# yang-song/score_sde_pytorch

Measured on AMD Instinct MI355X. Metric: pc_sampler_images_per_sec, higher is better.
Workload: dtype f32 via 3-way bf16 split, fp32 accumulate (the 1x1 / NIN / Linear GEMMs and the attention forward as exact-fp32 products on the BF16 matrix pipe, fp32 softmax; 3x3 convolutions and the attention backward on the fp32-MFMA kernels); 1 GPU; configs/ve/cifar10_ncsnpp_continuous PC sampler (reverse_diffusion+langevin), batch 256/GPU, N=1000, 32x32; 1 step = 1 PC iteration = 2 U-Net evaluations; batch_per_gpu=256, sde_steps=1000, state_finite=True, matrix_mode=bf16x6, parallelism=replicas x1 (no collectives)

## Files before the change

### include/ssde.h

```cpp
#ifndef SSDE_H_
#define SSDE_H_

#include <stddef.h>
#include <stdint.h>

#ifdef __cplusplus
extern "C" {
#endif

#define SSDE_ABI_VERSION 13

enum {
  SSDE_PRO_NONE = 0,
  SSDE_PRO_GN = 1,
  SSDE_PRO_GN_SILU = 2,
  SSDE_PRO_SILU = 3
};

typedef struct ssde_src {
  const float* p0;
  const float* p1;
  int32_t c0, c1;
  int32_t pro_mode;
  int32_t gn_groups;
// ... 38 lines not shown
  int64_t wino_ws_floats;
} ssde_conv_args;

enum { SSDE_CONVF_V_GIVEN = 1u,
       SSDE_CONVF_BF16X6 = 2u,
       SSDE_CONVF_NO_KSPLIT = 4u,
       SSDE_CONVF_BKC8 = 8u,
       SSDE_CONVF_GEMM_PIPE = 16u,
       SSDE_CONVF_NO_GEMM_PIPE = 32u,
       SSDE_CONVF_X6_BM64 = 64u,
       SSDE_CONVF_X6_PF2 = 128u,
       SSDE_CONVF_NO_SMALL_COUT = 256u,
       SSDE_CONVF_X6_WIDE = 512u,
       SSDE_CONVF_X6_NO_WIDE = 1024u,
       SSDE_CONVF_KSPLIT2 = 2048u,
       SSDE_CONVF_KSPLIT4 = 4096u };
enum { SSDE_TILE_AUTO = 0, SSDE_TILE_256x64 = 1, SSDE_TILE_128x64 = 2, SSDE_TILE_64x64 = 3, SSDE_TILE_256x32 = 4,
       SSDE_TILE_WINOGRAD = 5,
       SSDE_TILE_WINOGRAD4 = 6,
       SSDE_TILE_WINOGRAD4R = 9,
       SSDE_TILE_WINOGRAD4P = 10 };

typedef struct ssde_gn_stats_args {
  const float* p0; const float* p1; int32_t c0, c1;
  int32_t n, hw, groups; float eps;
  float* mean; float* rstd;
  float* scratch;
  int32_t slices;
  uint32_t flags;
} ssde_gn_stats_args;
enum { SSDE_GNSTATF_ANY_WIDTH = 1u };
// ... 227 lines not shown
} ssde_dsm_loss_args;

typedef struct ssde_sumsq_flat_args { const float* x; int64_t numel; float* partial; float* out; } ssde_sumsq_flat_args;
typedef struct ssde_adam_args {
  float* p; const float* g; float* m; float* v; float* ema;
  int64_t numel;
  const float* hyper;
  const float* gnorm_sq;
} ssde_adam_args;

typedef struct ssde_memset_args { void* dst; int64_t bytes; int32_t value; int32_t _pad0; } ssde_memset_args;

enum { SSDE_PACK_CONV3 = 1, SSDE_PACK_WINO3 = 2, SSDE_PACK_MATRIX = 3, SSDE_PACK_VECTOR = 4,
       SSDE_PACK_WINO4 = 5 ,
       SSDE_PACK_WINO4R = 6 ,
       SSDE_PACK_WINO4P = 7  };
typedef struct ssde_pack_desc {
  const float* src;
  const float* src2;
  float* dst;
  int32_t kind;
  int32_t cout, cin;
  int32_t cout_l, cin_l;
  int32_t flags;
  int32_t r_off, c_off;
  int64_t n;
} ssde_pack_desc;
typedef struct ssde_pack_args { const ssde_pack_desc* table; int32_t count; int32_t kind; int64_t max_n; } ssde_pack_args;
typedef struct ssde_axpy_args {
  const float* x; const float* gate; float* dst; int64_t numel; float alpha; int32_t acc;
} ssde_axpy_args;
// ... 188 lines not shown
```

### score_sde_pytorch_amd/_lib.py

```python
import ctypes as C
import os

_HERE = os.path.dirname(os.path.abspath(__file__))
LIB_PATH = os.environ.get("SSDE_LIB_PATH") or os.path.join(_HERE, "libssde_hip.so")
ABI_VERSION = 13

PRO_NONE, PRO_GN, PRO_GN_SILU, PRO_SILU = 0, 1, 2, 3
TILE_AUTO, TILE_256x64, TILE_128x64, TILE_64x64, TILE_256x32, TILE_WINOGRAD, TILE_WINOGRAD4 = 0, 1, 2, 3, 4, 5, 6
TILE_WINOGRAD4R = 9
TILE_WINOGRAD4P = 10
TILES_WINOGRAD4 = (TILE_WINOGRAD4, TILE_WINOGRAD4R, TILE_WINOGRAD4P)
CONVF_V_GIVEN, CONVF_BF16X6, CONVF_NO_KSPLIT, CONVF_BKC8, CONVF_GEMM_PIPE, CONVF_NO_GEMM_PIPE, CONVF_X6_BM64, CONVF_X6_PF2, \
    CONVF_NO_SMALL_COUT, CONVF_X6_WIDE, CONVF_X6_NO_WIDE, CONVF_KSPLIT2, CONVF_KSPLIT4 = 1, 2, 4, 8, 16, 32, 64, 128, 256, 512, 1024, 2048, 4096
WGRADF_DIRECT, WGRADF_F2, WGRADF_F4_FORCE, WGRADF_NO_STREAMK, WGRADF_NO_XCD_ORDER, WGRADF_1X1_CHUNKED, WGRADF_XVEC1 = 1, 2, 4, 8, 16, 32, 64
GNBWDF_THREE_KERNELS, GNBWDF_DEFER_PARAMS = 1, 2
(OP_CONV, OP_GN_STATS, OP_UPFIRDN, OP_ATTN, OP_EMBED, OP_TO_NHWC, OP_TO_NCHW, OP_BIAS_ACT, OP_SUMSQ,
 OP_RANDN, OP_LANGEVIN, OP_PREDICTOR, OP_FILL, OP_STEP_INC, OP_WGRAD, OP_COLSUM, OP_GN_BWD_REDUCE, OP_PROLOGUE_BWD,
 OP_ATTN_BWD, OP_PERTURB, OP_DSM_LOSS, OP_SUMSQ_FLAT, OP_ADAM, OP_MEMSET, OP_AXPY, OP_PACK, OP_PROJECT,
 OP_GN_FINALIZE, OP_PF_DRIFT, OP_HUTCH_DIV, OP_COLSUM_FINISH, OP_GN_BWD_FINISH, OP_GN_APPLY, OP_GN_APPLY_BWD) = range(1, 35)
GNSTATF_ANY_WIDTH = 1
FIRF_GENERAL, FIRF_TILED = 1, 2
FIR_MAX_TAPS = 16
FINISH_JOBS = 16
COLSUMF_DEFER = 1
PACK_CONV3, PACK_WINO3, PACK_MATRIX, PACK_VECTOR, PACK_WINO4, PACK_WINO4R, PACK_WINO4P = 1, 2, 3, 4, 5, 6, 7

_fp = C.c_void_p


class Src(C.Structure):
    _fields_ = [("p0", _fp), ("p1", _fp), ("c0", C.c_int32), ("c1", C.c_int32),
                ("pro_mode", C.c_int32), ("gn_groups", C.c_int32),
                ("gn_mean", _fp), ("gn_rstd", _fp), ("gn_gamma", _fp), ("gn_beta", _fp),
                ("drop_thresh", C.c_uint32), ("drop_scale", C.c_float), ("drop_seed", _fp),
                ("drop_salt", C.c_uint32), ("_pad", C.c_int32)]


class ConvArgs(C.Structure):
    _fields_ = [("main", Src), ("aux", Src), ("w_main", _fp), ("w_aux", _fp),
                ("n", C.c_int32), ("h_in", C.c_int32), ("w_in", C.c_int32),
# ... 439 lines not shown
```

### score_sde_pytorch_amd/csrc/backward.hip

```cpp
#include "ssde_common.h"

namespace {

inline unsigned grid_for(size_t total, int block = 256, unsigned cap = 256 * 16) {
  size_t b = (total + block - 1) / block;
  if (b < 1) b = 1;
  return (unsigned)(b > cap ? cap : b);
}

__global__ __launch_bounds__(256) void colsum_kernel(const float* __restrict__ g, int g_ld, int g_off, int hw, int c,
                                                     float scale, float* __restrict__ out, int out_ld, int out_off) {
  SSDE_LDS(smem);
  float4* red = reinterpret_cast<float4*>(smem);
  const int n = blockIdx.z, slices = gridDim.y, slice = blockIdx.y;
  const int cl = blockIdx.x * 64 + (threadIdx.x & 63);
  const int pl = threadIdx.x >> 6;
  const int col = g_off + cl * 4;
  const int per_slice = (hw + slices - 1) / slices;
  const int p0 = slice * per_slice, p1 = min(hw, p0 + per_slice);
  float4 s = make_float4(0.f, 0.f, 0.f, 0.f);
  if (cl * 4 < c && col + 4 <= g_ld) {
    const float* base = g + (size_t)n * hw * g_ld + col;
    int px = p0 + pl;
    for (; px + 12 < p1; px += 16) {
// ... 871 lines not shown
        const float u = (float)(t[a][0] * G[b][0] + t[a][1] * G[b][1] + t[a][2] * G[b][2]);
        if (kForm == 0) {
          d.dst[(((r * 8 + wv) * 9 + j) * 32 + (cs & 31)) * 4 + e] = u;
        } else if (kForm == 2) {
          d.dst[(((size_t)pos * nq + c4) * ((size_t)ntl * 64) + co) * 4 + e] = u;
        } else {
          const int lane = (e >> 1) * 32 + (cs & 31), half = cs >> 5;
          const int w = pos < 32 ? (pos >> 2) : 2 * (pos - 32) + half;
          const size_t base = (r * 8 + w) * (size_t)(9 * 32 * 4);
          d.dst[base + (pos < 32 ? ((pos & 3) * 64 + lane) * 4 + half * 2 + (e & 1) : 1024 + lane * 2 + (e & 1))] = u;
        }
      }
  }
}

__global__ __launch_bounds__(256) void pack_matrix_kernel(const ssde_pack_desc* __restrict__ table) {
  const ssde_pack_desc d = table[blockIdx.y];
  const int ld = (d.cout_l + 63) / 64 * 64;
  for (size_t idx = (size_t)blockIdx.x * 256 + threadIdx.x; idx < (size_t)d.n; idx += (size_t)gridDim.x * 256) {
    const int i = (int)(idx / d.cin), j = (int)(idx % d.cin);
    const int row = ((d.flags & 1) ? j : i) + d.r_off, col = ((d.flags & 1) ? i : j) + d.c_off;
    d.dst[((size_t)(col >> 3) * ld + row) * 8 + (col & 7)] = d.src[idx];
  }
}

__global__ __launch_bounds__(256) void pack_vector_kernel(const ssde_pack_desc* __restrict__ table) {
  const ssde_pack_desc d = table[blockIdx.y];
  for (size_t idx = (size_t)blockIdx.x * 256 + threadIdx.x; idx < (size_t)d.n; idx += (size_t)gridDim.x * 256)
    d.dst[d.r_off + idx] = d.src[idx] + (d.src2 ? d.src2[idx] : 0.f);
}

}

extern "C" int ssde_pack_weights(const ssde_pack_args* a, void* stream) {
  SSDE_REQUIRE(a && a->table && a->count > 0 && a->max_n > 0, "pack_weights: bad args");
  size_t bx = ((size_t)a->max_n + 255) / 256;
  if (bx > 256) bx = 256;
  const dim3 grid((unsigned)bx, (unsigned)a->count);
  hipStream_t st = static_cast<hipStream_t>(stream);
  switch (a->kind) {
    case SSDE_PACK_CONV3: hipLaunchKernelGGL(pack_conv3_kernel, grid, dim3(256), 0, st, a->table); break;
    case SSDE_PACK_WINO3: hipLaunchKernelGGL(pack_wino3_kernel, grid, dim3(256), 0, st, a->table); break;
    case SSDE_PACK_WINO4: hipLaunchKernelGGL(pack_wino4_kernel<0>, grid, dim3(256), 0, st, a->table); break;
    case SSDE_PACK_WINO4R: hipLaunchKernelGGL(pack_wino4_kernel<1>, grid, dim3(256), 0, st, a->table); break;
    case SSDE_PACK_WINO4P: hipLaunchKernelGGL(pack_wino4_kernel<2>, grid, dim3(256), 0, st, a->table); break;
    case SSDE_PACK_MATRIX: hipLaunchKernelGGL(pack_matrix_kernel, grid, dim3(256), 0, st, a->table); break;
    case SSDE_PACK_VECTOR: hipLaunchKernelGGL(pack_vector_kernel, grid, dim3(256), 0, st, a->table); break;
    default: ssde_set_error("pack_weights: unknown kind %d", a->kind); return SSDE_EINVAL;
  }
  SSDE_LAUNCH_CHECK();
  return SSDE_OK;
}
```

### score_sde_pytorch_amd/csrc/conv1x1.hip

```cpp
#include "ssde_common.h"

typedef float f32x16 __attribute__((ext_vector_type(16)));

#ifdef SSDE_GEMM_TRACE
__device__ unsigned long long* g_gemm_trace;
extern "C" int ssde_debug_gemm_trace(void* buf) {
  return hipMemcpyToSymbol(HIP_SYMBOL(g_gemm_trace), &buf, sizeof(buf)) == hipSuccess ? 0 : -5;
}
#define SSDE_GT(slot)                                                                  \
  do {                                                                                 \
    if (gt_on) g_gemm_trace[(slot)] = __builtin_amdgcn_s_memtime();                    \
  } while (0)
__device__ unsigned long long* g_gemm_wg_trace;
extern "C" int ssde_debug_gemm_wg_trace(void* buf) {
  return hipMemcpyToSymbol(HIP_SYMBOL(g_gemm_wg_trace), &buf, sizeof(buf)) == hipSuccess ? 0 : -5;
}
#define SSDE_GW(slot)                                                                                          \
  do {                                                                                                         \
    if (threadIdx.x == 0 && g_gemm_wg_trace != nullptr) {                                                      \
      g_gemm_wg_trace[(size_t)blockIdx.x * 4 + (slot)] = __builtin_amdgcn_s_memtime();                         \
      if ((slot) == 0) g_gemm_wg_trace[(size_t)blockIdx.x * 4 + 3] = __builtin_amdgcn_s_getreg((4 << 0) | (0 << 6) | (31 << 11)) | ((unsigned long long)__builtin_amdgcn_s_getreg((20 << 0) | (0 << 6) | (3 << 11)) << 32); \
    }                                                                                                          \
  } while (0)
#else
// ... 197 lines not shown
    SSDE_GT(41 + half * 2);
    __syncthreads();
    SSDE_GT(42 + half * 2);
  }
}

#ifndef SSDE_X6_PF2_OCC_LOSS
#define SSDE_X6_PF2_OCC_LOSS 1
#endif
constexpr int XBK = 16;
template <int kBM, int kBN = 128> struct X6 {
  static constexpr int kPlaneA = kBM * XBK * 2, kPlaneB = kBN * XBK * 2;
  static constexpr int kStageBytes = 3 * kPlaneA + 3 * kPlaneB;
  static constexpr int NA = kBM / 64;
  static constexpr int NBW = kBN / 64;
};

template <bool kGn, int kBM, int kPF, int kBN = 128>
__global__ __launch_bounds__(kThreads, kBN == 256 ? 2 : (kBM == 64 ? 4 : 3) - (kPF == 2 ? SSDE_X6_PF2_OCC_LOSS : 0)) void gemm1x1_bf16x6_kernel(const GemmParams p) {
  using X = X6<kBM, kBN>;
  constexpr int NA = X::NA, NB = X::NBW, NBW = X::NBW, RS = 64;
  SSDE_LDS(smem);
  char* lds = reinterpret_cast<char*>(smem);
  const int tid = threadIdx.x, wave = tid >> 6, lane = tid & 63;
  const int li = lane & 31, lh = lane >> 5;
  const int xcd = blockIdx.x & 7, lin = blockIdx.x >> 3;
  const int nt = lin % p.n_tiles, mt = (lin / p.n_tiles) * 8 + xcd;
#ifdef SSDE_GEMM_TRACE
  const bool gt_on = tid == 0 && blockIdx.x == 0 && g_gemm_trace != nullptr;
#endif
  SSDE_GT(0);
  if (mt >= p.m_tiles) return;
  SSDE_GW(0);
  const int m0 = mt * kBM, n0 = nt * kBN;
  const int wm0 = (wave >> 1) * (kBM / 2), wn0 = (wave & 1) * (kBN / 2);
  const ssde_src& s = p.src;
  SsdePro pro = ssde_pro_decode(s);
  pro.gn = kGn;
  const int Ctot = s.c0 + s.c1;
  const int cpg = kGn ? Ctot / s.gn_groups : 1;
  const int nst = (p.K + XBK - 1) / XBK;
  const int ncin8 = (p.K + 7) >> 3;

  const int f = tid & 3, r0 = tid >> 2;
  int arow[NA], aimg[NA];
  bool aok[NA];
#pragma unroll
  for (int i = 0; i < NA; ++i) {
    const int m = m0 + r0 + i * RS;
    aok[i] = m < p.M;
    arow[i] = aok[i] ? m : 0;
    aimg[i] = arow[i] / p.HW;
  }
  bool bok[NB];
#pragma unroll
  for (int i = 0; i < NB; ++i) bok[i] = (n0 + r0 + i * RS) < p.CoutPad;
  const float* bptr = p.wpk + ((size_t)n0 + r0) * 8 + (f & 1) * 4;

  struct ARegs { float4 av[NA]; };
  struct StageRegs {
    float4 bv[NB];
    float mu[NA], rs[NA];
    float4 gam, bet;
  };
  auto load_a = [&](int st, ARegs& A) __attribute__((always_inline)) {
    const int c_base = st * XBK;
    const bool second = c_base >= s.c0;
    const float* base = second ? s.p1 : s.p0;
    const int C = second ? s.c1 : s.c0;
    const int cthr = (second ? c_base - s.c0 : c_base) + f * 4;
    const float* ap = base + (c_base + f * 4 < p.K ? cthr : 0);
#pragma unroll
    for (int i = 0; i < NA; ++i) A.av[i] = *reinterpret_cast<const float4*>(ap + (size_t)arow[i] * C);
  };
  auto load_rest = [&](int st, StageRegs& R) __attribute__((always_inline)) {
    const int c_cur = st * XBK + f * 4;
    const int cin8 = min(st * 2 + (f >> 1), ncin8 - 1);
    const float* bp = bptr + (size_t)cin8 * p.CoutPad * 8;
#pragma unroll
    for (int i = 0; i < NB; ++i) R.bv[i] = *reinterpret_cast<const float4*>(bp + (bok[i] ? i * RS * 8 : 0));
    R.gam = make_float4(1.f, 1.f, 1.f, 1.f); R.bet = make_float4(0.f, 0.f, 0.f, 0.f);
#pragma unroll
    for (int i = 0; i < NA; ++i) { R.mu[i] = 0.f; R.rs[i] = 1.f; }
    if (kGn) {
      const int cg = c_cur < p.K ? c_cur : 0;
      R.gam = *reinterpret_cast<const float4*>(s.gn_gamma + cg);
      R.bet = *reinterpret_cast<const float4*>(s.gn_beta + cg);
#pragma unroll
      for (int i = 0; i < NA; ++i) {
        const int gi = aimg[i] * s.gn_groups + cg / cpg;
        R.mu[i] = s.gn_mean[gi];
        R.rs[i] = s.gn_rstd[gi];
      }
    }
  };
  auto store_stage = [&](int st, const ARegs& A, const StageRegs& R, char* buf) __attribute__((always_inline)) {
    const int cin8 = st * 2 + (f >> 1);
    const int c_cur = st * XBK + f * 4;
    const bool k_ok = c_cur < p.K;
    uint2 q0, q1, q2;
#pragma unroll
    for (int i = 0; i < NA; ++i) {
      float4 v = make_float4(0.f, 0.f, 0.f, 0.f);
      if (aok[i] && k_ok)
        v = ssde_pro_apply(A.av[i], R.mu[i], R.rs[i], R.gam, R.bet, (uint32_t)arow[i] * (uint32_t)Ctot + (uint32_t)c_cur, pro);
      char* d = buf + (r0 + i * RS) * (XBK * 2) + f * 8;
      ssde_split3(v, q0, q1, q2);
      *reinterpret_cast<uint2*>(d) = q0;
      *reinterpret_cast<uint2*>(d + X::kPlaneA) = q1;
      *reinterpret_cast<uint2*>(d + 2 * X::kPlaneA) = q2;
    }
#pragma unroll
    for (int i = 0; i < NB; ++i) {
      float4 w = make_float4(0.f, 0.f, 0.f, 0.f);
      if (bok[i] && cin8 < ncin8) w = R.bv[i];
      char* d = buf + 3 * X::kPlaneA + (r0 + i * RS) * (XBK * 2) + f * 8;
      ssde_split3(w, q0, q1, q2);
      *reinterpret_cast<uint2*>(d) = q0;
      *reinterpret_cast<uint2*>(d + X::kPlaneB) = q1;
      *reinterpret_cast<uint2*>(d + 2 * X::kPlaneB) = q2;
    }
  };

  f32x16 acc[NA][NBW];
#pragma unroll
  for (int a = 0; a < NA; ++a)
#pragma unroll
    for (int b = 0; b < NBW; ++b)
#pragma unroll
      for (int r = 0; r < 16; ++r) acc[a][b][r] = 0.f;
  const int aoff = (wm0 + li) * (XBK * 2) + lh * 16, boff = 3 * X::kPlaneA + (wn0 + li) * (XBK * 2) + lh * 16;
  auto mfma_stage = [&](const char* cur) __attribute__((always_inline)) {
    ssde_u32x4 A[NA][3];
#pragma unroll
    for (int q = 0; q < 3; ++q)
#pragma unroll
// ... 226 lines not shown
  auto run_tile = [&](int vb, f32x16 (&acc)[2][2], f32x16 (&old)[2][2]) __attribute__((always_inline)) {
    const int xcd = vb & 7, lin = vb >> 3;
    const int nt = lin % p.n_tiles, mt = (lin / p.n_tiles) * 8 + xcd;
    const int m0 = mt * BM, n0 = nt * BN;
    int arow[NI], aimg[NI];
    bool aok[NI], bok[NI];
#pragma unroll
    for (int i = 0; i < NI; ++i) {
      const int m = m0 + r0 + i * RS;
      aok[i] = m < p.M;
      arow[i] = aok[i] ? m : 0;
      aimg[i] = arow[i] / p.HW;
      bok[i] = (n0 + r0 + i * RS) < p.CoutPad;
    }
    const float* bptr = p.wpk + ((size_t)n0 + r0) * 8 + (f & 1) * 4;
    float4 av[NI], bv[NI];
    float mu[NI] = {0.f, 0.f}, rs[NI] = {1.f, 1.f};
    float4 gam = make_float4(1.f, 1.f, 1.f, 1.f), bet = make_float4(0.f, 0.f, 0.f, 0.f);
    auto load_stage = [&](int st) __attribute__((always_inline)) {
      const int c_base = st * KB;
      const bool second = c_base >= s.c0;
      const float* base = second ? s.p1 : s.p0;
      const int C = second ? s.c1 : s.c0;
      const int cthr = (second ? c_base - s.c0 : c_base) + f * 4;
      const int c_cur = c_base + f * 4;
      const float* ap = base + (c_cur < p.K ? cthr : 0);
#pragma unroll
      for (int i = 0; i < NI; ++i) av[i] = *reinterpret_cast<const float4*>(ap + (size_t)arow[i] * C);
      const int cin8 = min(st * 2 + (f >> 1), ncin8 - 1);
      const float* bp = bptr + (size_t)cin8 * p.CoutPad * 8;
#pragma unroll
      for (int i = 0; i < NI; ++i) bv[i] = *reinterpret_cast<const float4*>(bp + (bok[i] ? i * RS * 8 : 0));
      if (kGn) {
        const int cg = c_cur < p.K ? c_cur : 0;
        gam = *reinterpret_cast<const float4*>(s.gn_gamma + cg);
        bet = *reinterpret_cast<const float4*>(s.gn_beta + cg);
#pragma unroll
        for (int i = 0; i < NI; ++i) {
          const int gi = aimg[i] * s.gn_groups + cg / cpg;
          mu[i] = s.gn_mean[gi];
          rs[i] = s.gn_rstd[gi];
        }
      }
    };
    auto store_stage = [&](int st, char* buf) __attribute__((always_inline)) {
      const int cin8 = st * 2 + (f >> 1), c_cur = st * KB + f * 4;
      const bool k_ok = c_cur < p.K;
#pragma unroll
      for (int i = 0; i < NI; ++i) {
        float4 v = make_float4(0.f, 0.f, 0.f, 0.f);
        if (aok[i] && k_ok)
          v = ssde_pro_apply(av[i], mu[i], rs[i], gam, bet, (uint32_t)arow[i] * (uint32_t)Ctot + (uint32_t)c_cur, pro);
        float4 w = make_float4(0.f, 0.f, 0.f, 0.f);
        if (bok[i] && cin8 < ncin8) w = bv[i];
        if constexpr (kX6) {
          using X = X6<128>;
          uint2 q0, q1, q2;
          char* d = buf + (r0 + i * RS) * (KB * 2) + f * 8;
          ssde_split3(v, q0, q1, q2);
          *reinterpret_cast<uint2*>(d) = q0;
          *reinterpret_cast<uint2*>(d + X::kPlaneA) = q1;
          *reinterpret_cast<uint2*>(d + 2 * X::kPlaneA) = q2;
          ssde_split3(w, q0, q1, q2);
          *reinterpret_cast<uint2*>(d + 3 * X::kPlaneA) = q0;
          *reinterpret_cast<uint2*>(d + 3 * X::kPlaneA + X::kPlaneB) = q1;
          *reinterpret_cast<uint2*>(d + 3 * X::kPlaneA + 2 * X::kPlaneB) = q2;
        } else {
          float* fb = reinterpret_cast<float*>(buf);
          float* d = fb + (r0 + i * RS) * LDK + f * 4;
          *reinterpret_cast<float2*>(d) = make_float2(v.x, v.y);
          *reinterpret_cast<float2*>(d + 2) = make_float2(v.z, v.w);
          float* e = fb + (BM + r0 + i * RS) * LDK + f * 4;
          *reinterpret_cast<float2*>(e) = make_float2(w.x, w.y);
          *reinterpret_cast<float2*>(e + 2) = make_float2(w.z, w.w);
        }
      }
    };
    auto mfma_stage = [&](const char* cur) __attribute__((always_inline)) {
      if constexpr (kX6) {
        using X = X6<128>;
        const int aoff = (wm0 + li) * (KB * 2) + lh * 16, boff = 3 * X::kPlaneA + (wn0 + li) * (KB * 2) + lh * 16;
        ssde_u32x4 A[2][3], B[2][3];
#pragma unroll
        for (int q = 0; q < 3; ++q)
#pragma unroll
          for (int a = 0; a < 2; ++a) {
            A[a][q] = *reinterpret_cast<const ssde_u32x4*>(cur + aoff + q * X::kPlaneA + a * 32 * (KB * 2));
            B[a][q] = *reinterpret_cast<const ssde_u32x4*>(cur + boff + q * X::kPlaneB + a * 32 * (KB * 2));
          }
// ... 92 lines not shown
  g->gn = s.pro_mode == SSDE_PRO_GN || s.pro_mode == SSDE_PRO_GN_SILU;
  SSDE_REQUIRE(a->w_aux && a->dst, "conv1x1: null weights / destination");
  GemmParams& p = g->p;
  p.src = s; p.wpk = a->w_aux;
  p.M = a->n * a->h_out * a->w_out; p.HW = a->h_out * a->w_out; p.K = s.c0 + s.c1;
  p.Cout = a->c_out; p.CoutPad = ssde_cdiv(a->c_out, 64) * 64;
  p.m_tiles = ssde_cdiv(p.M, BM); p.n_tiles = ssde_cdiv(a->c_out, BN);
  ssde_fill_epilogue(p, a);
  const bool gn_ok = a->c_out % 4 == 0 && (p.HW % 64 == 0 || (p.HW >= 8 && p.HW < 64 && 64 % p.HW == 0));
  SSDE_REQUIRE(!a->gn_part || gn_ok, "conv1x1: GroupNorm partials need H*W %% 64 == 0 or a power of two in 8..32");
  pl->gn_slices = !gn_ok ? 0 : p.HW % 64 == 0 ? (p.HW / 64) * 4 : 4;
  pl->ws_floats = 0;
  p.lHW = ssde_ilog2(p.HW);
  p.gn_entries = p.HW >= 64 ? a->n * (p.HW / 64) : a->n;
  const bool x6 = g->x6 = (a->flags & SSDE_CONVF_BF16X6) != 0;
  {
    const int total = ssde_cdiv(p.m_tiles, 8) * 8 * p.n_tiles;
    const int wgs = (2 * ssde_num_cus() + 7) / 8 * 8;
    const bool pipe_ok = !(a->flags & SSDE_CONVF_NO_GEMM_PIPE) && a->c_out % 4 == 0 && (!a->gn_part || p.HW % 64 == 0) && (!a->chan_add || p.HW % 8 == 0);
    const bool wide_first = a->c_out >= 512 && a->c_out % 256 == 0 && !(a->flags & (SSDE_CONVF_X6_NO_WIDE | SSDE_CONVF_X6_BM64 | SSDE_CONVF_X6_PF2)) &&
                            (long long)ssde_cdiv(p.M, 128) * (a->c_out / 256) >= 2ll * ssde_num_cus();
    const bool pays = x6 && p.K >= 512 && (long long)p.m_tiles * p.n_tiles > wgs && !wide_first;
    g->pipe = pipe_ok && x6 && (pays || (a->flags & SSDE_CONVF_GEMM_PIPE));
    if (g->pipe) {
      pl->lds_bytes = 2 * X6<128>::kStageBytes + 4 * kSlabFloats * 4;
      g->grid = total < wgs ? total : wgs;
      return SSDE_OK;
    }
  }
  int xbm = 128, xpf = 1, xbn = BN;
// ... 25 lines not shown
bool ssde_conv1x1_wants(const ssde_conv_args* a) {
  if (a->ksize != 0 || a->aux.p0 == nullptr || a->tile != SSDE_TILE_AUTO) return false;
  const long long M = (long long)a->n * a->h_out * a->w_out;
  return a->c_out >= 96 && M >= 128 && M < (1ll << 31);
}

int ssde_conv1x1_plan(const ssde_conv_args* a, ssde_conv_plan* pl) {
  GemmPlan g;
  return gemm_plan(a, &g, pl);
}

int ssde_conv1x1_launch(const ssde_conv_args* a, hipStream_t st) {
  GemmPlan g;
  ssde_conv_plan pl;
  if (int rc = gemm_plan(a, &g, &pl)) return rc;
  const int lds = pl.lds_bytes;
  const bool gn = g.gn;
  if (g.pipe) return gn ? gemm_go<gemm1x1_pipe_kernel<true, true>>(g, lds, st) : gemm_go<gemm1x1_pipe_kernel<false, true>>(g, lds, st);
  if (!g.x6) return gn ? gemm_go<gemm1x1_kernel<true>>(g, lds, st) : gemm_go<gemm1x1_kernel<false>>(g, lds, st);
  if (g.xbn == 256) return gn ? gemm_go<gemm1x1_bf16x6_kernel<true, 128, 1, 256>>(g, lds, st) : gemm_go<gemm1x1_bf16x6_kernel<false, 128, 1, 256>>(g, lds, st);
  if (g.xbm == 128 && g.xpf == 1) return gn ? gemm_go<gemm1x1_bf16x6_kernel<true, 128, 1>>(g, lds, st) : gemm_go<gemm1x1_bf16x6_kernel<false, 128, 1>>(g, lds, st);
  if (g.xbm == 128) return gn ? gemm_go<gemm1x1_bf16x6_kernel<true, 128, 2>>(g, lds, st) : gemm_go<gemm1x1_bf16x6_kernel<false, 128, 2>>(g, lds, st);
  if (g.xpf == 1) return gn ? gemm_go<gemm1x1_bf16x6_kernel<true, 64, 1>>(g, lds, st) : gemm_go<gemm1x1_bf16x6_kernel<false, 64, 1>>(g, lds, st);
  return gn ? gemm_go<gemm1x1_bf16x6_kernel<true, 64, 2>>(g, lds, st) : gemm_go<gemm1x1_bf16x6_kernel<false, 64, 2>>(g, lds, st);
}
```

### score_sde_pytorch_amd/engine.py

```python
import ctypes as C
import math
import os
from typing import Callable, NamedTuple

import numpy as np
import torch

from . import _lib as L

_FLT = 4
INV_SQRT2 = float(1.0 / np.sqrt(2.0))

FC_OTHER, FC_CONV3, FC_CONV1, FC_ATTN, FC_GN, FC_FIR = 0, 1, 2, 3, 4, 5

W4P_MIN_BATCH = 16


class Buf:
    __slots__ = ("shape", "numel", "name", "persistent", "tensor", "first", "last")

    def __init__(self, shape, name="", persistent=False):
        self.shape = tuple(int(s) for s in shape)
        self.numel = int(np.prod(self.shape))
        self.name = name
# ... 111 lines not shown
                    free.append(b.tensor)
        self.blocks = blocks
        self.arena_bytes = sum(t.numel() for t in blocks) * _FLT
        ops, classes, flops, starts = [], [], [], []
        for si, (kind, fields, fclass, fl) in enumerate(self.specs):
            starts.append(len(ops))
            if si in fused_fir:
                if fused_fir[si] is None:
                    continue
                fields = dict(fields, dst2=fused_fir[si])
            for sub_fields, sub_class, sub_fl in _expand(kind, fields, fclass, fl):
                args = L.ARGS[kind]()
                _fill(args, sub_fields)
                if kind in _ROUTE and "flags" not in sub_fields:
                    args.flags = _ROUTE[kind]()
                ops.append(L.make_op(kind, args, sub_class))
                classes.append(sub_class)
                flops.append(sub_fl)
        prog = Program(L.op_array(ops), classes, flops, self)
        prog.spec_start = starts + [len(ops)]
        return prog


def _fir_pairs(specs):
    out = {}
    if os.environ.get("SSDE_FUSE_FIR", "1") == "0":
        return out
    same = ("n", "h_in", "w_in", "c", "h_out", "w_out", "up", "down", "pad0", "pad1", "kh", "kw", "k")
    for i in range(len(specs) - 1):
        (k0, f0, _, _), (k1, f1, _, _) = specs[i], specs[i + 1]
# ... 178 lines not shown
    c4, nt = (w.shape[1] + 3) // 4, (w.shape[0] + 63) // 64
    v = _wino4_u(w).reshape(nt, 2, 32, c4, 2, 2, 36)
    fp = v[..., :32].reshape(nt, 2, 32, c4, 2, 2, 8, 4).permute(3, 0, 6, 7, 4, 2, 1, 5).reshape(c4, nt, 8, 4 * 64 * 4)
    hp = v[..., 32:].permute(3, 0, 6, 1, 4, 2, 5).reshape(c4, nt, 8, 64 * 2)
    return torch.cat([fp, hp], dim=3).contiguous()


def pack_wino4p_weight(w):
    return _wino4_u(w).unflatten(1, (-1, 4)).permute(3, 1, 0, 2).contiguous()


def pack_matrix(w):
    return pack_conv_weight(w.reshape(w.shape[0], w.shape[1], 1, 1))


class Conv3Route(NamedTuple):
    name: str
    tile: int
    pack_kind: int
    pack: Callable
    takes_v: bool
    needs_ws: bool


DIRECT = Conv3Route("direct", L.TILE_AUTO, L.PACK_CONV3, pack_conv_weight, False, False)
F2 = Conv3Route("f2", L.TILE_WINOGRAD, L.PACK_WINO3, pack_wino_weight, False, False)
F4 = Conv3Route("f4", L.TILE_WINOGRAD4, L.PACK_WINO4, pack_wino4_weight, True, False)
F4R = Conv3Route("f4r", L.TILE_WINOGRAD4R, L.PACK_WINO4R, pack_wino4r_weight, True, False)
F4P = Conv3Route("f4p", L.TILE_WINOGRAD4P, L.PACK_WINO4P, pack_wino4p_weight, False, True)
CONV3_ROUTES = (DIRECT, F2, F4, F4R, F4P)
# ... 65 lines not shown
                w = w.to(torch.float32)
                w = w.t() if tr else w.reshape(w.shape[0], -1)
                ms.append(w)
            m = torch.cat(ms, dim=0) if len(ms) > 1 else ms[0]
            if cin_pad and m.shape[1] < cin_pad:
                m = torch.nn.functional.pad(m, (0, cin_pad - m.shape[1]))
            return m
        rows, desc = 0, []
        for p_, tr in parts:
            n_rows = p_.shape[1] if tr else p_.shape[0]
            cin = p_.shape[0] if tr else int(np.prod(p_.shape[1:]))
            desc.append(dict(param=p_, row0=rows, rows=n_rows, transpose=tr))
            rows += n_rows
        meta = dict(kind="matrix", sources=params, logical=logical, parts=desc, cin_store=cin,
                    dims=(rows, max(cin, cin_pad or 0)))
        recipe = [dict(kind=L.PACK_MATRIX, src=d["param"], cout=d["param"].shape[0], cin=int(np.prod(d["param"].shape[1:])),
                       cout_l=rows, cin_l=0, flags=int(d["transpose"]), r_off=d["row0"], c_off=0, n="src") for d in desc]
        return self.add(params, lambda *ws: pack_matrix(logical(*ws)), meta, recipe)

    def vector(self, params, mode="cat", pad_to=None):
        def fn(*vs):
            vs = [v.to(torch.float32) for v in vs]
            x = torch.cat(vs) if mode == "cat" else sum(vs[1:], vs[0])
            if pad_to and x.numel() < pad_to:
                x = torch.nn.functional.pad(x, (0, pad_to - x.numel()))
            return x.clone()
        off, desc = 0, []
        for p_ in params:
            desc.append(dict(param=p_, off=0 if mode == "sum" else off, n=p_.numel()))
            off += p_.numel()
        if mode == "sum":
            assert len(params) == 2
            recipe = [dict(kind=L.PACK_VECTOR, src=params[0], src2=params[1], r_off=0, n="src")]
        else:
            recipe = [dict(kind=L.PACK_VECTOR, src=d["param"], r_off=d["off"], n="src") for d in desc]
        return self.add(params, fn, dict(kind="vector", mode=mode, sources=list(params), parts=desc), recipe)

    def derived(self, packed, route=None):
        meta = self.meta[id(packed)]
        key = (id(packed), route)
        if key not in self.meta:
            cout_l, cin_l = meta["dims"]
            if meta["kind"] == "conv3":
                p_ = meta["sources"][0]
                fn = lambda w: route.pack(w.permute(1, 0, 2, 3).flip(2, 3))
                recipe = [dict(kind=route.pack_kind, src=p_, cout=p_.shape[0], cin=p_.shape[1],
                               cout_l=cin_l, cin_l=cout_l, flags=1, n="dst")]
            else:
                fn = lambda m: pack_matrix(m.t().contiguous())
                recipe = [dict(kind=L.PACK_MATRIX, src=d["param"], cout=d["param"].shape[0], cin=int(np.prod(d["param"].shape[1:])),
                               cout_l=cin_l, cin_l=0, flags=int(not d["transpose"]), r_off=0, c_off=d["row0"], n="src")
                          for d in meta["parts"]]
            self.meta[key] = self.add(meta["sources"], lambda *ws: fn(meta["logical"](*ws)), None, recipe)
        return self.meta[key]

    def _source_addresses(self):
        return tuple(s.data_ptr() for e in self.entries if e.recipe is not None for s in e.sources)

    def _build_tables(self):
        descs = {}
        for e in self.entries:
            packed, recipe = e.packed, e.recipe
            if recipe is None:
                continue
            for r in recipe:
                d = L.PackDesc()
                src = r["src"]
                d.src, d.dst, d.kind = src.data_ptr(), packed.data_ptr(), r["kind"]
# ... 662 lines not shown
```

### score_sde_pytorch_amd/hipops.py

```python
import ctypes as C

import numpy as np
import torch

from . import _lib as L
from .engine import F4R, conv3_route_of_tile, pack_conv_weight, pack_matrix, wino4_v_floats


def _stream():
    return C.c_void_p(torch.cuda.current_stream().cuda_stream)


def _need_cuda(*ts):
    for t in ts:
        if t is not None and not t.is_cuda:
            raise RuntimeError("score_sde_pytorch_amd HIP op called with a %s tensor (no CPU fallback)" % t.device.type)


def _p(t):
    return None if t is None else t.data_ptr()


def _fill_src(s, t, t2=None, pro=L.PRO_NONE, gn=None):
    s.p0, s.c0 = _p(t), t.shape[-1]
# ... 51 lines not shown
    _fill_drop(a.src, drop)
    sums = torch.empty(n, gn[4], 2, device=x.device)
    scratch = torch.empty(n * slices * c * 2, device=x.device)
    dgamma, dbeta = torch.empty(c, device=x.device), torch.empty(c, device=x.device)
    a.acc0, a.acc1 = int(g0 is not None), int(g1 is not None)
    g0 = torch.empty_like(x) if g0 is None else g0
    g1 = (torch.empty_like(x2) if g1 is None else g1) if x2 is not None else None
    a.dy, a.n, a.hw, a.sums, a.dgamma, a.dbeta, a.scratch, a.slices = _p(dy), n, hw, _p(sums), _p(dgamma), _p(dbeta), _p(scratch), slices
    a.g0, a.g1 = _p(g0), _p(g1)
    L.check(L.load().ssde_gn_apply_bwd(C.byref(a), _stream()), "ssde_gn_apply_bwd")
    return g0, g1, dgamma, dbeta


def conv2d(x=None, weight=None, bias=None, stride=1, pad=1, x2=None, pro=L.PRO_NONE, gn=None,
           aux=None, aux2=None, aux_weight=None, aux_pro=L.PRO_NONE, aux_gn=None,
           chan_add=None, resid=None, scale=1.0, tile=L.TILE_AUTO, out_hw=None, flags=None, pad_end=0):
    _need_cuda(x, aux, resid)
    a = L.ConvArgs()
    keep = []
    route = conv3_route_of_tile(tile)
    if x is not None:
        n, h_in, w_in = x.shape[0], x.shape[1], x.shape[2]
        c_out = weight.shape[0]
        h_out = (h_in + 2 * pad + pad_end - 3) // stride + 1
        w_out = (w_in + 2 * pad + pad_end - 3) // stride + 1
        if out_hw is not None:
            h_out, w_out = out_hw
        _fill_src(a.main, x, x2, pro, gn)
        wp = route.pack(weight.to(x.device)); keep.append(wp)
        if route is F4R:
            wv = torch.empty(wino4_v_floats(n, h_in, w_in, x.shape[-1] + (x2.shape[-1] if x2 is not None else 0)), device=x.device)
            keep.append(wv)
            a.wino_v = _p(wv)
        a.w_main, a.ksize, a.stride, a.pad, a.h_in, a.w_in = _p(wp), 3, stride, pad, h_in, w_in
        a.pad_end = pad_end
    else:
        n, h_out, w_out = aux.shape[0], aux.shape[1], aux.shape[2]
        c_out = aux_weight.shape[0]
        a.ksize, a.stride, a.pad = 0, 1, 0
    if aux is not None:
        _fill_src(a.aux, aux, aux2, aux_pro, aux_gn)
        wa = pack_matrix(aux_weight.to(aux.device)); keep.append(wa)
        a.w_aux = _p(wa)
    dev = (x if x is not None else aux).device
    dst = torch.empty(n, h_out, w_out, c_out, device=dev)
    a.n, a.h_out, a.w_out, a.c_out, a.tile = n, h_out, w_out, c_out, tile
    a.bias = _p(bias)
    if chan_add is not None:
        a.chan_add, a.chan_add_ld = _p(chan_add), chan_add.shape[-1]
    a.resid, a.out_scale, a.dst = _p(resid), scale, _p(dst)
    a.flags = L.conv_route_flags() if flags is None else flags
    if route.needs_ws:
        need = int(L.load().ssde_conv_ws_floats(C.byref(a)))
        L.check(min(need, 0), "ssde_conv_ws_floats")
        ws = torch.empty(need, device=dev); keep.append(ws)
        a.wino_ws, a.wino_ws_floats = _p(ws), need
    L.check(L.load().ssde_conv2d(C.byref(a), _stream()), "ssde_conv2d")
    return dst


def upfirdn2d_nhwc(x, kernel, up=1, down=1, pad=(0, 0), pro=L.PRO_NONE, gn=None, dual=False, accumulate_into=None, flags=0):
    _need_cuda(x)
    n, h, w, c = x.shape
    kh, kw = kernel.shape
    if not (1 <= kh <= L.FIR_MAX_TAPS and 1 <= kw <= L.FIR_MAX_TAPS):
        raise ValueError("upfirdn2d: a %dx%d kernel; at most %d taps per axis" % (kh, kw, L.FIR_MAX_TAPS))
# ... 297 lines not shown
```

Before: 5.589 images/s.

## Pre-split 1x1 GEMM weights into bf16x3 planes at pack time

The weight packer now also writes three bf16 split planes (hi, mid, lo) in a per-stage layout next to the fp32 packed matrix. The bf16x6 1x1 GEMM kernels load those planes with 16-byte vector reads and copy them straight into LDS, so they no longer run the per-stage ssde_split3 on weights inside the hot loop. This cuts ALU work and simplifies the B-operand staging, but adds weight memory, a flag that must be set when packing, and a hard error when it is missing.

```diff
diff --git a/include/ssde.h b/include/ssde.h
--- a/include/ssde.h
+++ b/include/ssde.h
@@ -76,7 +76,8 @@
        SSDE_CONVF_X6_WIDE = 512u,
        SSDE_CONVF_X6_NO_WIDE = 1024u,
        SSDE_CONVF_KSPLIT2 = 2048u,
-       SSDE_CONVF_KSPLIT4 = 4096u };
+       SSDE_CONVF_KSPLIT4 = 4096u,
+       SSDE_CONVF_W_AUX_X6 = 8192u };
 enum { SSDE_TILE_AUTO = 0, SSDE_TILE_256x64 = 1, SSDE_TILE_128x64 = 2, SSDE_TILE_64x64 = 3, SSDE_TILE_256x32 = 4,
        SSDE_TILE_WINOGRAD = 5,
        SSDE_TILE_WINOGRAD4 = 6,
@@ -334,7 +335,8 @@
 enum { SSDE_PACK_CONV3 = 1, SSDE_PACK_WINO3 = 2, SSDE_PACK_MATRIX = 3, SSDE_PACK_VECTOR = 4,
        SSDE_PACK_WINO4 = 5 ,
        SSDE_PACK_WINO4R = 6 ,
-       SSDE_PACK_WINO4P = 7  };
+       SSDE_PACK_WINO4P = 7 ,
+       SSDE_PACK_MATRIX_X6 = 8 };
 typedef struct ssde_pack_desc {
   const float* src;
   const float* src2;
diff --git a/score_sde_pytorch_amd/_lib.py b/score_sde_pytorch_amd/_lib.py
--- a/score_sde_pytorch_amd/_lib.py
+++ b/score_sde_pytorch_amd/_lib.py
@@ -12,6 +12,7 @@
 TILES_WINOGRAD4 = (TILE_WINOGRAD4, TILE_WINOGRAD4R, TILE_WINOGRAD4P)
 CONVF_V_GIVEN, CONVF_BF16X6, CONVF_NO_KSPLIT, CONVF_BKC8, CONVF_GEMM_PIPE, CONVF_NO_GEMM_PIPE, CONVF_X6_BM64, CONVF_X6_PF2, \
     CONVF_NO_SMALL_COUT, CONVF_X6_WIDE, CONVF_X6_NO_WIDE, CONVF_KSPLIT2, CONVF_KSPLIT4 = 1, 2, 4, 8, 16, 32, 64, 128, 256, 512, 1024, 2048, 4096
+CONVF_W_AUX_X6 = 8192
 WGRADF_DIRECT, WGRADF_F2, WGRADF_F4_FORCE, WGRADF_NO_STREAMK, WGRADF_NO_XCD_ORDER, WGRADF_1X1_CHUNKED, WGRADF_XVEC1 = 1, 2, 4, 8, 16, 32, 64
 GNBWDF_THREE_KERNELS, GNBWDF_DEFER_PARAMS = 1, 2
 (OP_CONV, OP_GN_STATS, OP_UPFIRDN, OP_ATTN, OP_EMBED, OP_TO_NHWC, OP_TO_NCHW, OP_BIAS_ACT, OP_SUMSQ,
@@ -23,7 +24,7 @@
 FIR_MAX_TAPS = 16
 FINISH_JOBS = 16
 COLSUMF_DEFER = 1
-PACK_CONV3, PACK_WINO3, PACK_MATRIX, PACK_VECTOR, PACK_WINO4, PACK_WINO4R, PACK_WINO4P = 1, 2, 3, 4, 5, 6, 7
+PACK_CONV3, PACK_WINO3, PACK_MATRIX, PACK_VECTOR, PACK_WINO4, PACK_WINO4R, PACK_WINO4P, PACK_MATRIX_X6 = 1, 2, 3, 4, 5, 6, 7, 8
 
 _fp = C.c_void_p
 
diff --git a/score_sde_pytorch_amd/csrc/backward.hip b/score_sde_pytorch_amd/csrc/backward.hip
--- a/score_sde_pytorch_amd/csrc/backward.hip
+++ b/score_sde_pytorch_amd/csrc/backward.hip
@@ -909,13 +909,24 @@
   }
 }
 
+template <bool kX6>
 __global__ __launch_bounds__(256) void pack_matrix_kernel(const ssde_pack_desc* __restrict__ table) {
   const ssde_pack_desc d = table[blockIdx.y];
   const int ld = (d.cout_l + 63) / 64 * 64;
+  uint16_t* planes = reinterpret_cast<uint16_t*>(d.dst + (size_t)((d.cin_l + 7) >> 3) * ld * 8);
   for (size_t idx = (size_t)blockIdx.x * 256 + threadIdx.x; idx < (size_t)d.n; idx += (size_t)gridDim.x * 256) {
     const int i = (int)(idx / d.cin), j = (int)(idx % d.cin);
     const int row = ((d.flags & 1) ? j : i) + d.r_off, col = ((d.flags & 1) ? i : j) + d.c_off;
-    d.dst[((size_t)(col >> 3) * ld + row) * 8 + (col & 7)] = d.src[idx];
+    const float w = d.src[idx];
+    d.dst[((size_t)(col >> 3) * ld + row) * 8 + (col & 7)] = w;
+    if (kX6) {
+      uint2 q0, q1, q2;
+      ssde_split3(make_float4(w, 0.f, 0.f, 0.f), q0, q1, q2);
+      uint16_t* o = planes + ((size_t)(col >> 4) * 3 * ld + row) * 16 + (col & 15);
+      o[0] = (uint16_t)q0.x;
+      o[(size_t)ld * 16] = (uint16_t)q1.x;
+      o[(size_t)ld * 32] = (uint16_t)q2.x;
+    }
   }
 }
 
@@ -939,7 +950,8 @@
     case SSDE_PACK_WINO4: hipLaunchKernelGGL(pack_wino4_kernel<0>, grid, dim3(256), 0, st, a->table); break;
     case SSDE_PACK_WINO4R: hipLaunchKernelGGL(pack_wino4_kernel<1>, grid, dim3(256), 0, st, a->table); break;
     case SSDE_PACK_WINO4P: hipLaunchKernelGGL(pack_wino4_kernel<2>, grid, dim3(256), 0, st, a->table); break;
-    case SSDE_PACK_MATRIX: hipLaunchKernelGGL(pack_matrix_kernel, grid, dim3(256), 0, st, a->table); break;
+    case SSDE_PACK_MATRIX: hipLaunchKernelGGL(pack_matrix_kernel<false>, grid, dim3(256), 0, st, a->table); break;
+    case SSDE_PACK_MATRIX_X6: hipLaunchKernelGGL(pack_matrix_kernel<true>, grid, dim3(256), 0, st, a->table); break;
     case SSDE_PACK_VECTOR: hipLaunchKernelGGL(pack_vector_kernel, grid, dim3(256), 0, st, a->table); break;
     default: ssde_set_error("pack_weights: unknown kind %d", a->kind); return SSDE_EINVAL;
   }
diff --git a/score_sde_pytorch_amd/csrc/conv1x1.hip b/score_sde_pytorch_amd/csrc/conv1x1.hip
--- a/score_sde_pytorch_amd/csrc/conv1x1.hip
+++ b/score_sde_pytorch_amd/csrc/conv1x1.hip
@@ -235,12 +235,13 @@
   static constexpr int kStageBytes = 3 * kPlaneA + 3 * kPlaneB;
   static constexpr int NA = kBM / 64;
   static constexpr int NBW = kBN / 64;
+  static constexpr int NBV = kPlaneB / (kThreads * 16);
 };
 
 template <bool kGn, int kBM, int kPF, int kBN = 128>
 __global__ __launch_bounds__(kThreads, kBN == 256 ? 2 : (kBM == 64 ? 4 : 3) - (kPF == 2 ? SSDE_X6_PF2_OCC_LOSS : 0)) void gemm1x1_bf16x6_kernel(const GemmParams p) {
   using X = X6<kBM, kBN>;
-  constexpr int NA = X::NA, NB = X::NBW, NBW = X::NBW, RS = 64;
+  constexpr int NA = X::NA, NB = X::NBV, NBW = X::NBW, RS = 64;
   SSDE_LDS(smem);
   char* lds = reinterpret_cast<char*>(smem);
   const int tid = threadIdx.x, wave = tid >> 6, lane = tid & 63;
@@ -261,7 +262,6 @@
   const int Ctot = s.c0 + s.c1;
   const int cpg = kGn ? Ctot / s.gn_groups : 1;
   const int nst = (p.K + XBK - 1) / XBK;
-  const int ncin8 = (p.K + 7) >> 3;
 
   const int f = tid & 3, r0 = tid >> 2;
   int arow[NA], aimg[NA];
@@ -274,13 +274,18 @@
     aimg[i] = arow[i] / p.HW;
   }
   bool bok[NB];
-#pragma unroll
-  for (int i = 0; i < NB; ++i) bok[i] = (n0 + r0 + i * RS) < p.CoutPad;
-  const float* bptr = p.wpk + ((size_t)n0 + r0) * 8 + (f & 1) * 4;
+  int bofs[NB];
+#pragma unroll
+  for (int i = 0; i < NB; ++i) {
+    bok[i] = (n0 + (tid >> 1) + i * 128) < p.CoutPad;
+    bofs[i] = bok[i] ? tid * 16 + i * 4096 : 0;
+  }
+  const size_t wplane = (size_t)p.CoutPad * (XBK * 2);
+  const char* bptr = reinterpret_cast<const char*>(p.wpk) + (size_t)n0 * (XBK * 2);
 
   struct ARegs { float4 av[NA]; };
   struct StageRegs {
-    float4 bv[NB];
+    ssde_u32x4 bv[3][NB];
     float mu[NA], rs[NA];
     float4 gam, bet;
   };
@@ -296,10 +301,11 @@
   };
   auto load_rest = [&](int st, StageRegs& R) __attribute__((always_inline)) {
     const int c_cur = st * XBK + f * 4;
-    const int cin8 = min(st * 2 + (f >> 1), ncin8 - 1);
-    const float* bp = bptr + (size_t)cin8 * p.CoutPad * 8;
-#pragma unroll
-    for (int i = 0; i < NB; ++i) R.bv[i] = *reinterpret_cast<const float4*>(bp + (bok[i] ? i * RS * 8 : 0));
+    const char* bp = bptr + (size_t)st * 3 * wplane;
+#pragma unroll
+    for (int q = 0; q < 3; ++q)
+#pragma unroll
+      for (int i = 0; i < NB; ++i) R.bv[q][i] = *reinterpret_cast<const ssde_u32x4*>(bp + q * wplane + bofs[i]);
     R.gam = make_float4(1.f, 1.f, 1.f, 1.f); R.bet = make_float4(0.f, 0.f, 0.f, 0.f);
 #pragma unroll
     for (int i = 0; i < NA; ++i) { R.mu[i] = 0.f; R.rs[i] = 1.f; }
@@ -316,7 +322,6 @@
     }
   };
   auto store_stage = [&](int st, const ARegs& A, const StageRegs& R, char* buf) __attribute__((always_inline)) {
-    const int cin8 = st * 2 + (f >> 1);
     const int c_cur = st * XBK + f * 4;
     const bool k_ok = c_cur < p.K;
     uint2 q0, q1, q2;
@@ -332,15 +337,12 @@
       *reinterpret_cast<uint2*>(d + 2 * X::kPlaneA) = q2;
     }
 #pragma unroll
-    for (int i = 0; i < NB; ++i) {
-      float4 w = make_float4(0.f, 0.f, 0.f, 0.f);
-      if (bok[i] && cin8 < ncin8) w = R.bv[i];
-      char* d = buf + 3 * X::kPlaneA + (r0 + i * RS) * (XBK * 2) + f * 8;
-      ssde_split3(w, q0, q1, q2);
-      *reinterpret_cast<uint2*>(d) = q0;
-      *reinterpret_cast<uint2*>(d + X::kPlaneB) = q1;
-      *reinterpret_cast<uint2*>(d + 2 * X::kPlaneB) = q2;
-    }
+    for (int q = 0; q < 3; ++q)
+#pragma unroll
+      for (int i = 0; i < NB; ++i) {
+        const ssde_u32x4 z = {0u, 0u, 0u, 0u};
+        *reinterpret_cast<ssde_u32x4*>(buf + 3 * X::kPlaneA + q * X::kPlaneB + tid * 16 + i * 4096) = bok[i] ? R.bv[q][i] : z;
+      }
   };
 
   f32x16 acc[NA][NBW];
@@ -597,6 +599,10 @@
       bok[i] = (n0 + r0 + i * RS) < p.CoutPad;
     }
     const float* bptr = p.wpk + ((size_t)n0 + r0) * 8 + (f & 1) * 4;
+    const bool xok = (n0 + (tid >> 1)) < p.CoutPad;
+    const size_t wplane = (size_t)p.CoutPad * (KB * 2);
+    const char* xptr = reinterpret_cast<const char*>(p.wpk) + (size_t)n0 * (KB * 2) + (xok ? tid * 16 : 0);
+    ssde_u32x4 xv[3];
     float4 av[NI], bv[NI];
     float mu[NI] = {0.f, 0.f}, rs[NI] = {1.f, 1.f};
     float4 gam = make_float4(1.f, 1.f, 1.f, 1.f), bet = make_float4(0.f, 0.f, 0.f, 0.f);
@@ -610,10 +616,15 @@
       const float* ap = base + (c_cur < p.K ? cthr : 0);
 #pragma unroll
       for (int i = 0; i < NI; ++i) av[i] = *reinterpret_cast<const float4*>(ap + (size_t)arow[i] * C);
-      const int cin8 = min(st * 2 + (f >> 1), ncin8 - 1);
-      const float* bp = bptr + (size_t)cin8 * p.CoutPad * 8;
-#pragma unroll
-      for (int i = 0; i < NI; ++i) bv[i] = *reinterpret_cast<const float4*>(bp + (bok[i] ? i * RS * 8 : 0));
+      if constexpr (kX6) {
+#pragma unroll
+        for (int q = 0; q < 3; ++q) xv[q] = *reinterpret_cast<const ssde_u32x4*>(xptr + ((size_t)st * 3 + q) * wplane);
+      } else {
+        const int cin8 = min(st * 2 + (f >> 1), ncin8 - 1);
+        const float* bp = bptr + (size_t)cin8 * p.CoutPad * 8;
+#pragma unroll
+        for (int i = 0; i < NI; ++i) bv[i] = *reinterpret_cast<const float4*>(bp + (bok[i] ? i * RS * 8 : 0));
+      }
       if (kGn) {
         const int cg = c_cur < p.K ? c_cur : 0;
         gam = *reinterpret_cast<const float4*>(s.gn_gamma + cg);
@@ -627,15 +638,13 @@
       }
     };
     auto store_stage = [&](int st, char* buf) __attribute__((always_inline)) {
-      const int cin8 = st * 2 + (f >> 1), c_cur = st * KB + f * 4;
+      const int c_cur = st * KB + f * 4;
       const bool k_ok = c_cur < p.K;
 #pragma unroll
       for (int i = 0; i < NI; ++i) {
         float4 v = make_float4(0.f, 0.f, 0.f, 0.f);
         if (aok[i] && k_ok)
           v = ssde_pro_apply(av[i], mu[i], rs[i], gam, bet, (uint32_t)arow[i] * (uint32_t)Ctot + (uint32_t)c_cur, pro);
-        float4 w = make_float4(0.f, 0.f, 0.f, 0.f);
-        if (bok[i] && cin8 < ncin8) w = bv[i];
         if constexpr (kX6) {
           using X = X6<128>;
           uint2 q0, q1, q2;
@@ -644,11 +653,9 @@
           *reinterpret_cast<uint2*>(d) = q0;
           *reinterpret_cast<uint2*>(d + X::kPlaneA) = q1;
           *reinterpret_cast<uint2*>(d + 2 * X::kPlaneA) = q2;
-          ssde_split3(w, q0, q1, q2);
-          *reinterpret_cast<uint2*>(d + 3 * X::kPlaneA) = q0;
-          *reinterpret_cast<uint2*>(d + 3 * X::kPlaneA + X::kPlaneB) = q1;
-          *reinterpret_cast<uint2*>(d + 3 * X::kPlaneA + 2 * X::kPlaneB) = q2;
         } else {
+          float4 w = make_float4(0.f, 0.f, 0.f, 0.f);
+          if (bok[i] && st * 2 + (f >> 1) < ncin8) w = bv[i];
           float* fb = reinterpret_cast<float*>(buf);
           float* d = fb + (r0 + i * RS) * LDK + f * 4;
           *reinterpret_cast<float2*>(d) = make_float2(v.x, v.y);
@@ -656,6 +663,15 @@
           float* e = fb + (BM + r0 + i * RS) * LDK + f * 4;
           *reinterpret_cast<float2*>(e) = make_float2(w.x, w.y);
           *reinterpret_cast<float2*>(e + 2) = make_float2(w.z, w.w);
+        }
+      }
+      if constexpr (kX6) {
+        using X = X6<128>;
+        static_assert(X::NBV == 1, "one 16-byte piece of a weight plane per thread");
+#pragma unroll
+        for (int q = 0; q < 3; ++q) {
+          const ssde_u32x4 z = {0u, 0u, 0u, 0u};
+          *reinterpret_cast<ssde_u32x4*>(buf + 3 * X::kPlaneA + q * X::kPlaneB + tid * 16) = xok ? xv[q] : z;
         }
       }
     };
@@ -778,6 +794,7 @@
   p.lHW = ssde_ilog2(p.HW);
   p.gn_entries = p.HW >= 64 ? a->n * (p.HW / 64) : a->n;
   const bool x6 = g->x6 = (a->flags & SSDE_CONVF_BF16X6) != 0;
+  if (x6) p.wpk = a->w_aux + (size_t)((p.K + 7) >> 3) * p.CoutPad * 8;
   {
     const int total = ssde_cdiv(p.m_tiles, 8) * 8 * p.n_tiles;
     const int wgs = (2 * ssde_num_cus() + 7) / 8 * 8;
@@ -833,6 +850,8 @@
   GemmPlan g;
   ssde_conv_plan pl;
   if (int rc = gemm_plan(a, &g, &pl)) return rc;
+  SSDE_REQUIRE(!g.x6 || (a->flags & SSDE_CONVF_W_AUX_X6),
+               "conv1x1: a bf16x6 GEMM reads its weights as bf16 planes -- pack w_aux as SSDE_PACK_MATRIX_X6 and set SSDE_CONVF_W_AUX_X6");
   const int lds = pl.lds_bytes;
   const bool gn = g.gn;
   if (g.pipe) return gn ? gemm_go<gemm1x1_pipe_kernel<true, true>>(g, lds, st) : gemm_go<gemm1x1_pipe_kernel<false, true>>(g, lds, st);
diff --git a/score_sde_pytorch_amd/engine.py b/score_sde_pytorch_amd/engine.py
--- a/score_sde_pytorch_amd/engine.py
+++ b/score_sde_pytorch_amd/engine.py
@@ -149,6 +149,8 @@
                 _fill(args, sub_fields)
                 if kind in _ROUTE and "flags" not in sub_fields:
                     args.flags = _ROUTE[kind]()
+                if kind == L.OP_CONV and getattr(sub_fields.get("w_aux"), "_ssde_x6", False):
+                    args.flags |= L.CONVF_W_AUX_X6
                 ops.append(L.make_op(kind, args, sub_class))
                 classes.append(sub_class)
                 flops.append(sub_fl)
@@ -357,6 +359,30 @@
     return pack_conv_weight(w.reshape(w.shape[0], w.shape[1], 1, 1))
 
 
+def split3_bf16(w):
+    w = w.to(torch.float32).contiguous()
+    top = lambda x: (x.view(torch.int32) & -65536).view(torch.float32)
+    r1 = w - top(w)
+    r2 = r1 - top(r1)
+    return [(x.contiguous().view(torch.int32) >> 16) & 0xFFFF for x in (w, r1, r2)]
+
+
+def matrix_x6_floats(cout, cin):
+    ld = (cout + 63) // 64 * 64
+    return (cin + 7) // 8 * ld * 8, (cin + 15) // 16 * ld * 24
+
+
+def pack_matrix_x6(w):
+    cout, cin = w.shape
+    ld, nst = (cout + 63) // 64 * 64, (cin + 15) // 16
+    full = torch.zeros(ld, nst * 16, dtype=torch.float32, device=w.device)
+    full[:cout, :cin] = w.detach().to(torch.float32)
+    pieces = torch.stack(split3_bf16(full), 0).reshape(3, ld, nst, 8, 2)
+    words = pieces[..., 0] | (pieces[..., 1] << 16)
+    planes = words.permute(2, 0, 1, 3).contiguous().view(torch.float32).reshape(-1)
+    return torch.cat([pack_matrix(w).reshape(-1), planes])
+
+
 class Conv3Route(NamedTuple):
     name: str
     tile: int
@@ -452,9 +478,14 @@
             rows += n_rows
         meta = dict(kind="matrix", sources=params, logical=logical, parts=desc, cin_store=cin,
                     dims=(rows, max(cin, cin_pad or 0)))
-        recipe = [dict(kind=L.PACK_MATRIX, src=d["param"], cout=d["param"].shape[0], cin=int(np.prod(d["param"].shape[1:])),
-                       cout_l=rows, cin_l=0, flags=int(d["transpose"]), r_off=d["row0"], c_off=0, n="src") for d in desc]
-        return self.add(params, lambda *ws: pack_matrix(logical(*ws)), meta, recipe)
+        recipe = [dict(kind=L.PACK_MATRIX_X6, src=d["param"], cout=d["param"].shape[0], cin=int(np.prod(d["param"].shape[1:])),
+                       cout_l=rows, cin_l=meta["dims"][1], flags=int(d["transpose"]), r_off=d["row0"], c_off=0, n="src") for d in desc]
+        return self._x6(self.add(params, lambda *ws: pack_matrix_x6(logical(*ws)), meta, recipe))
+
+    @staticmethod
+    def _x6(packed):
+        packed._ssde_x6 = True
+        return packed
 
     def vector(self, params, mode="cat", pad_to=None):
         def fn(*vs):
@@ -485,11 +516,13 @@
                 recipe = [dict(kind=route.pack_kind, src=p_, cout=p_.shape[0], cin=p_.shape[1],
                                cout_l=cin_l, cin_l=cout_l, flags=1, n="dst")]
             else:
-                fn = lambda m: pack_matrix(m.t().contiguous())
-                recipe = [dict(kind=L.PACK_MATRIX, src=d["param"], cout=d["param"].shape[0], cin=int(np.prod(d["param"].shape[1:])),
-                               cout_l=cin_l, cin_l=0, flags=int(not d["transpose"]), r_off=0, c_off=d["row0"], n="src")
+                fn = lambda m: pack_matrix_x6(m.t().contiguous())
+                recipe = [dict(kind=L.PACK_MATRIX_X6, src=d["param"], cout=d["param"].shape[0], cin=int(np.prod(d["param"].shape[1:])),
+                               cout_l=cin_l, cin_l=cout_l, flags=int(not d["transpose"]), r_off=0, c_off=d["row0"], n="src")
                           for d in meta["parts"]]
             self.meta[key] = self.add(meta["sources"], lambda *ws: fn(meta["logical"](*ws)), None, recipe)
+            if meta["kind"] != "conv3":
+                self._x6(self.meta[key])
         return self.meta[key]
 
     def _source_addresses(self):
diff --git a/score_sde_pytorch_amd/hipops.py b/score_sde_pytorch_amd/hipops.py
--- a/score_sde_pytorch_amd/hipops.py
+++ b/score_sde_pytorch_amd/hipops.py
@@ -4,7 +4,7 @@
 import torch
 
 from . import _lib as L
-from .engine import F4R, conv3_route_of_tile, pack_conv_weight, pack_matrix, wino4_v_floats
+from .engine import F4R, conv3_route_of_tile, pack_conv_weight, pack_matrix, pack_matrix_x6, wino4_v_floats
 
 
 def _stream():
@@ -89,7 +89,7 @@
 
 def conv2d(x=None, weight=None, bias=None, stride=1, pad=1, x2=None, pro=L.PRO_NONE, gn=None,
            aux=None, aux2=None, aux_weight=None, aux_pro=L.PRO_NONE, aux_gn=None,
-           chan_add=None, resid=None, scale=1.0, tile=L.TILE_AUTO, out_hw=None, flags=None, pad_end=0):
+           chan_add=None, resid=None, scale=1.0, tile=L.TILE_AUTO, out_hw=None, flags=None, pad_end=0, aux_packed=None, resid_post=0):
     _need_cuda(x, aux, resid)
     a = L.ConvArgs()
     keep = []
@@ -115,7 +115,7 @@
         a.ksize, a.stride, a.pad = 0, 1, 0
     if aux is not None:
         _fill_src(a.aux, aux, aux2, aux_pro, aux_gn)
-        wa = pack_matrix(aux_weight.to(aux.device)); keep.append(wa)
+        wa = aux_packed if aux_packed is not None else pack_matrix_x6(aux_weight.to(aux.device)); keep.append(wa)
         a.w_aux = _p(wa)
     dev = (x if x is not None else aux).device
     dst = torch.empty(n, h_out, w_out, c_out, device=dev)
@@ -123,8 +123,8 @@
     a.bias = _p(bias)
     if chan_add is not None:
         a.chan_add, a.chan_add_ld = _p(chan_add), chan_add.shape[-1]
-    a.resid, a.out_scale, a.dst = _p(resid), scale, _p(dst)
-    a.flags = L.conv_route_flags() if flags is None else flags
+    a.resid, a.resid_post, a.out_scale, a.dst = _p(resid), resid_post, scale, _p(dst)
+    a.flags = (L.conv_route_flags() if flags is None else flags) | (L.CONVF_W_AUX_X6 if aux is not None else 0)
     if route.needs_ws:
         need = int(L.load().ssde_conv_ws_floats(C.byref(a)))
         L.check(min(need, 0), "ssde_conv_ws_floats")
```

Result: no change. 5.587 images/s (median of 4 runs) (-0.0%).
